# cudagu/aero-gnn

Measured on AMD Instinct MI355X. Metric: million edge-updates/sec, 1M-node/6M-edge mesh, 1->8 MI355X, higher is better.
Workload: dtype bf16; 1 GPU; BSMS-MGN 4-scale U-Net train step (fwd+MSE+bwd+allreduce+Adam), 1000000 nodes / 5996000 edges per GPU; model=BiStridedMeshGraphNet(H=128, n_hid=2, processor_size=15, stride=2, concat_trick), mode=train, global_batch=1, parallelism=dp1

## Files before the change

### aero-gnn_amd/aerognn/_lib.py

```python
from __future__ import annotations

import ctypes as C
import os

_HERE = os.path.dirname(os.path.abspath(__file__))
LIB_PATH = os.environ.get("AEROGNN_LIB") or os.path.join(_HERE, "libaerognn.so")

MAX_LIN = 8
MAX_SEG = 3
F32, BF16, F16, F64 = 0, 1, 2, 3
SEG_PLAIN, SEG_GATHER, SEG_SUM, SEG_MEAN = 0, 1, 2, 3
OPT_RESIDENT = 0

vp = C.c_void_p
i32 = C.c_int


class Seg(C.Structure):
    _fields_ = [("kind", i32), ("k", i32), ("ld", i32), ("_pad", i32),
                ("ptr", vp), ("index", vp), ("store", vp)]


ACT = {"relu": 0, "gelu": 1, "silu": 2, "tanh": 3}

# ... 34 lines not shown

class WgradBatch(C.Structure):
    _fields_ = [("n", i32), ("_pad", i32), ("d", WgradDesc * MAX_WGRAD)]


class WecArgs(C.Structure):
    _fields_ = [("n", i32), ("e", i32), ("dtype", i32), ("out_dim", i32), ("hid", i32), ("pos_dim", i32),
                ("pos_ld", i32), ("mean", i32),
                ("rowptr", vp), ("src", vp), ("dst", vp), ("perm", vp), ("rowptr_src", vp), ("perm_src", vp),
                ("pos", vp), ("pab", vp), ("tx", vp), ("w1c", vp), ("w2", vp),
                ("w_in", vp), ("w_out", vp), ("out", vp), ("dout", vp), ("gw", vp), ("s_csc", vp), ("dh", vp),
                ("dpa", vp), ("dpb", vp), ("dtx", vp), ("dw_in", vp), ("partial", vp)]


class EdgeBwdArgs(C.Structure):
    _fields_ = [("rows", i32), ("nblk", i32), ("wpk", vp * 4), ("bias", vp * 4), ("ln_g", vp), ("e", vp),
                ("proj", vp), ("src", vp), ("dst", vp), ("g", vp), ("g2", vp), ("de", vp), ("g0", vp),
                ("dw_partial", vp), ("db_partial", vp), ("ln_partial", vp), ("stamps", vp),
                ("a1", vp), ("stats", vp), ("scratch", vp), ("wtpk0", vp),
                ("xk", i32), ("xld", i32)]


class EdgeFwdArgs(C.Structure):
    _fields_ = [("rows", i32), ("nblk", i32), ("wpk", vp * 4), ("bias", vp * 4), ("ln_g", vp), ("ln_b", vp),
                ("e", vp), ("proj", vp), ("src", vp), ("dst", vp), ("out", vp), ("act", vp * 3), ("hpre", vp),
                ("stats", vp)]


class PackDesc(C.Structure):
    _fields_ = [("src", vp), ("dst", vp), ("src_dtype", i32), ("dst_dtype", i32),
                ("rows", i32), ("cols", i32), ("trans", i32), ("ld", i32),
                ("row_off", i32), ("col_off", i32), ("dst_rows", i32), ("dst_cols", i32)]


class F64Seg(C.Structure):
    _fields_ = [("a", vp), ("aidx", vp), ("lda", i32), ("k", i32), ("w", vp), ("ldw", i32), ("transw", i32)]


class F64GemmArgs(C.Structure):
    _fields_ = [("rows", i32), ("n", i32), ("nseg", i32), ("_pad", i32), ("seg", F64Seg * 3), ("bias", vp),
                ("add", vp * 2), ("add_idx", vp * 2), ("add_ld", i32 * 2), ("mask", vp), ("mask_ld", i32),
                ("relu", i32), ("out", vp), ("out_ld", i32), ("mask_act", i32), ("pre_out", vp),
                ("pre_ld", i32), ("_pad3", i32)]


class F64WgradArgs(C.Structure):
    _fields_ = [("rows", i32), ("m", i32), ("k", i32), ("_pad", i32), ("g", vp), ("ldg", i32), ("_pad1", i32),
                ("x", vp), ("ldx", i32), ("_pad2", i32), ("xidx", vp), ("dw", vp), ("ldw", i32), ("_pad3", i32),
                ("db", vp)]


_lib = None

LAUNCHES = ("agn_pack", "agn_mlp_forward", "agn_mlp_backward", "agn_reduce_partials", "agn_wgrad", "agn_colsum",
            "agn_segment_sum", "agn_segment_sum2", "agn_gather_rows", "agn_radix_sort_u64", "agn_row_ptr", "agn_row_ptr_i64",
            "agn_iota_keys", "agn_level_index",
            "agn_exclusive_scan_i32", "agn_pool_sort_keys", "agn_pool_assign", "agn_pool_edge_candidates",
            "agn_pool_edge_sort", "agn_pool_edge_emit", "agn_bfs_distance", "agn_center_seed", "agn_maxdeg_seed",
            "agn_bistride_select", "agn_index_map", "agn_subgraph_edges", "agn_scatter_rows", "agn_wec_forward",
            "agn_wec_backward", "agn_edge_features", "agn_node_features", "agn_normalize", "agn_col_stats", "agn_collate",
            "agn_segment_max", "agn_segment_max_backward", "agn_edge_bwd_fused", "agn_encoder_bwd_fused", "agn_wgrad_reduce",
            "agn_edge_forward32",
            "agn_proj_forward", "agn_proj_backward")


class AeroGNNError(RuntimeError):
    pass


class _Lib:

    def __init__(self, cdll):
        self._cdll = cdll
        for name in LAUNCHES:
            if hasattr(cdll, name):
                setattr(self, name, _timed_launch(getattr(cdll, name), name[4:]))

    def __getattr__(self, name):
        return getattr(self._cdll, name)


def _timed_launch(f, tag):
    from . import core

    def call(*args):
        prof = core.PROF
        if prof is None or core._TIMED_DEPTH:
            return f(*args)
        import torch
        s = torch.cuda.Event(enable_timing=True)
        s.record()
        rc = f(*args)
        e = torch.cuda.Event(enable_timing=True)
        e.record()
        prof.append((tag, None, s, e))
        return rc
    return call


def lib():
    global _lib
    if _lib is None:
        if not os.path.exists(LIB_PATH):
            raise AeroGNNError(
                f"{LIB_PATH} not found: build it with `make -C aero-gnn_amd/csrc` "
                "(or __graft_entry__.build()); the aerognn hot path has no CPU fallback")
        L = C.CDLL(LIB_PATH)
        sig = {
            "agn_version": (i32, []),
            "agn_error_string": (C.c_char_p, [i32]),
            "agn_set_option": (i32, [i32, i32]),
            "agn_packed_bytes": (C.c_size_t, [i32, i32, i32]),
            "agn_pack": (i32, [vp, i32, i32, vp]),
            "agn_mlp_forward": (i32, [C.POINTER(MlpFwdArgs), vp]),
            "agn_mlp_bwd_nwaves": (i32, [i32]),
            "agn_mlp_backward": (i32, [C.POINTER(MlpBwdArgs), vp]),
            "agn_reduce_partials": (i32, [vp, i32, i32, vp, vp]),
            "agn_wgrad_nsplit": (i32, [i32, i32]),
            "agn_wgrad_partial_floats": (C.c_size_t, [i32, i32, i32]),
            "agn_wgrad": (i32, [C.POINTER(WgradBatch), i32, i32, vp]),
            "agn_wgrad_plan": (i32, [C.POINTER(WgradBatch)]),
            "agn_colsum": (i32, [vp, i32, i32, vp, i32, vp, vp]),
            "agn_segment_sum": (i32, [i32, i32, i32, vp, vp, vp, i32, vp, i32, i32, vp]),
            "agn_segment_sum2": (i32, [i32, i32, i32, vp, i32, vp, vp, vp, i32, vp, vp, vp, i32, vp, i32, vp]),
            "agn_gather_rows": (i32, [i32, i32, i32, vp, vp, i32, vp, vp, i32, vp, i32, vp]),
            "agn_segment_max": (i32, [i32, i32, i32, vp, vp, vp, i32, vp, i32, vp, vp]),
            "agn_segment_max_backward": (i32, [i32, i32, i32, vp, vp, i32, vp, i32, vp]),
            "agn_radix_sort_temp_bytes": (C.c_size_t, [i32]),
            "agn_radix_sort_u64": (i32, [vp, vp, i32, i32, vp, vp, vp, vp]),
            "agn_row_ptr": (i32, [vp, i32, i32, vp, vp]),
            "agn_row_ptr_i64": (i32, [vp, i32, i32, vp, vp]),
            "agn_iota_keys": (i32, [i32, vp, vp, vp, vp, vp]),
            "agn_level_index": (i32, [i32, vp, C.c_int64, vp, vp, vp, vp, vp, vp, vp]),
            "agn_scan_temp_bytes": (C.c_size_t, [i32]),
            "agn_exclusive_scan_i32": (i32, [vp, vp, i32, vp, vp, vp]),
            "agn_pool_sort_keys": (i32, [i32, vp, vp, i32, vp, vp, vp]),
            "agn_pool_assign": (i32, [i32, i32, i32, vp, vp, vp, vp, i32, vp, vp, vp, vp, vp]),
            "agn_pool_edge_candidates": (i32, [i32, vp, vp, vp, vp, vp]),
            "agn_pool_edge_sort": (i32, [i32, vp, vp, vp, vp, vp, vp, vp, vp, vp, vp, vp]),
            "agn_pool_edge_emit": (i32, [i32, vp, vp, vp, vp, vp, vp, vp, vp, vp, vp, i32, vp]),
            "agn_bfs_work_ints": (C.c_size_t, [i32]),
            "agn_bfs_distance": (i32, [vp, vp, i32, i32, vp, vp, C.POINTER(i32), vp]),
            "agn_center_seed": (i32, [vp, i32, i32, i32, vp, vp]),
            "agn_maxdeg_seed": (i32, [vp, i32, vp, vp]),
            "agn_compact_work_ints": (C.c_size_t, [i32]),
            "agn_bistride_select": (i32, [vp, i32, vp, C.POINTER(i32), vp, vp]),
            "agn_index_map": (i32, [vp, i32, i32, vp, vp]),
            "agn_subgraph_edges": (i32, [vp, vp, i32, vp, vp, vp, C.POINTER(i32), vp, vp]),
            "agn_scatter_rows": (i32, [i32, i32, i32, vp, vp, i32, vp, i32, vp]),
            "agn_wec_blocks": (i32, [i32]),
            "agn_edge_bwd_blocks": (i32, [i32]),
            "agn_edge_bwd_scratch_bytes": (C.c_size_t, [i32]),
            "agn_edge_features": (i32, [i32, C.c_int64, i32, vp, vp, i32, vp, vp, vp, vp, vp]),
            "agn_normalize": (i32, [i32, i32, vp, i32, vp, vp, vp, i32, i32, vp]),
            "agn_col_stats_temp_bytes": (C.c_size_t, [i32, i32]),
            "agn_col_stats": (i32, [i32, i32, vp, i32, vp, vp, C.c_float, vp, vp]),
            "agn_collate": (i32, [i32, C.c_int64, C.c_int64, vp, vp, vp, vp, vp]),
            "agn_edge_bwd_fused": (i32, [C.POINTER(EdgeBwdArgs), vp]),
            "agn_encoder_bwd_fused": (i32, [C.POINTER(EdgeBwdArgs), vp]),
            "agn_edge_fwd32_blocks": (i32, [i32]),
            "agn_edge_forward32": (i32, [C.POINTER(EdgeFwdArgs), vp]),
            "agn_debug_node32_launches": (C.c_long, []),
            "agn_debug_enc32_launches": (C.c_long, []),
            "agn_debug_dec32_launches": (C.c_long, []),
            "agn_debug_node32_bwd_launches": (C.c_long, []),
            "agn_debug_dec32_bwd_launches": (C.c_long, []),
            "agn_fault_status": (i32, [C.POINTER(i32), i32]),
            "agn_fault_status_async": (i32, [vp, vp]),
            "agn_debug_set_fault": (i32, [i32]),
            "agn_wgrad_reduce": (i32, [C.POINTER(WgradBatch), i32, vp]),
            "agn_proj_forward": (i32, [i32, vp, i32, vp, vp, vp, i32, vp]),
            "agn_proj_backward": (i32, [i32, vp, vp, i32, vp, vp, i32, vp]),
            "agn_wec_forward": (i32, [C.POINTER(WecArgs), vp]),
            "agn_wec_backward": (i32, [C.POINTER(WecArgs), vp]),
# ... 39 lines not shown
```

### aero-gnn_amd/aerognn/core.py

```python
from __future__ import annotations

import ctypes as C

import torch

from . import _lib as L
from ._lib import check, ptr


def stream():
    return C.c_void_p(torch.cuda.current_stream().cuda_stream)


PROF = None
_TIMED_DEPTH = 0


class _Timed:
    __slots__ = ("tag", "cost", "s", "on")

    def __init__(self, tag, cost):
        self.tag, self.cost = tag, cost
        self.on = False

# ... 496 lines not shown
        self.tag = tag

    def add(self, G, X, dw, db=None, xidx=None):
        assert G.dtype == X.dtype and logical_rows(G) == (logical_rows(X) if xidx is None else xidx.numel())
        assert dw.dtype == torch.float32 and dw.stride(1) == 1
        assert xidx is None or (xidx.dtype == torch.int32 and not is_tiled(X))
        self.items.append((G, X, dw, db, xidx))

    def run(self):
        lib = L.lib()
        plain = [it for it in self.items if it[4] is None]
        gath = [it for it in self.items if it[4] is not None]
        chunks = [grp[i:i + L.MAX_WGRAD] for grp in (plain, gath) for i in range(0, len(grp), L.MAX_WGRAD)]
        for chunk in chunks:
            dev = chunk[0][0].device
            live = []
            for G, X, dw, db, xi in chunk:
                if logical_rows(G) == 0:
                    dw.zero_()
                    if db is not None:
                        db.zero_()
                else:
                    live.append((G, X, dw, db, xi))
            if not live:
                continue
            b = L.WgradBatch()
            b.n = len(live)
            for j, (G, X, dw, db, xi) in enumerate(live):
                b.d[j] = L.WgradDesc(ptr(G), ptr(X), G.stride(0), X.stride(0), G.shape[1], X.shape[1], logical_rows(G),
                                     dw.stride(0), None, None, ptr(dw), ptr(db), int(is_tiled(G)), int(is_tiled(X)), 0, 0,
                                     ptr(xi))
            check(lib.agn_wgrad_plan(C.byref(b)), "wgrad_plan")
            sizes = [int(lib.agn_wgrad_partial_floats(G.shape[1], X.shape[1], b.d[j].nsplit))
                     for j, (G, X, _, _, _) in enumerate(live)]
            bsz = [b.d[j].nsplit * ((G.shape[1] + 127) // 128) * 128 if db is not None else 0
                   for j, (G, _, _, db, _) in enumerate(live)]
            scratch = torch.empty(sum(sizes) + sum(bsz), dtype=torch.float32, device=dev)
            o = 0
            for j, (G, X, dw, db, _) in enumerate(live):
                b.d[j].dw_partial = ptr(scratch[o:o + sizes[j]])
                o += sizes[j]
                if db is not None:
                    b.d[j].db_partial = ptr(scratch[o:o + bsz[j]])
                    o += bsz[j]
            s_el = live[0][0].element_size()
            io = sum(logical_rows(G) * (G.shape[1] + X.shape[1]) * s_el + 4 * G.shape[1] * (X.shape[1] + 1)
                     for G, X, _, _, _ in live)
            fl = sum(2.0 * logical_rows(G) * G.shape[1] * X.shape[1] for G, X, _, _, _ in live)
            with timed(self.tag, (0.0, fl, io)):
                check(lib.agn_wgrad(C.byref(b), dt_code(live[0][0].dtype), 0, stream()), "wgrad")
        self.items = []


def alg8d_edge(E, N, H, s, bwd=False):
    return (2 if bwd else 1) * (E * (2 * s * H + 8) + N * 2 * s * H)


def alg8d_node(N, H, s, bwd=False, proj=False):
    return (2 if bwd else 1) * N * 3 * s * H * (2 if (bwd and proj) else 1)


def with_alg(alg, impl):
    return (alg, impl[1], impl[0])


def mask_bytes(H):
    return 8 * max(1, (H + 63) // 64)


def cost_edge_fwd(E, N, H, s, nlin, train, a1_saves=False):
    per = 2 * H * s + 8 + ((nlin - 1) * (H * s + mask_bytes(H)) + H * s + 8 if train else 0)
    per += (H * s + 8) if a1_saves else 0
    return E * per + N * 2 * H * s, 2 * E * H * H * nlin


def cost_node_fwd(E, N, H, s, nlin, train):
    per = 2 * H * s + 8 + ((nlin - 1) * (H * s + mask_bytes(H)) + 2 * H * s + 8 if train else 0)
    return N * per + E * H * s, 2 * N * H * (2 * H + (nlin - 1) * H)


def cost_proj(N, H, s):
    return N * 3 * H * s, 2 * N * H * 2 * H


def cost_edge_bwd(E, N, H, s, nlin):
    per = H * s + H * s + (nlin - 1) * mask_bytes(H) + H * s + 8 + nlin * H * s + H * s + 4
    return E * per + N * H * s, 2 * E * H * H * nlin


def cost_edge_fwd_cat(E, N, H, s, nlin, train):
    per = 4 * H * s + 8 + ((nlin - 1) * (H * s + mask_bytes(H)) + H * s + 8 if train else 0)
    return E * per, 2 * E * H * (3 * H + (nlin - 1) * H)


def cost_edge_bwd_cat(E, N, H, s, nlin):
    per = H * s + H * s + (nlin - 1) * mask_bytes(H) + H * s + 8 + nlin * H * s + 3 * H * s + 4
    return E * per + N * H * s, 2 * E * H * (3 * H + (nlin - 1) * H)


def cost_wec_fwd(E, N, out, s, hid=64):
    return E * (12 + hid * s + out * s + 24 + s) + N * (8 + hid * s + out * s), E * (2 * hid + 2 * out + 16)


def cost_wec_bwd(E, N, out, s, hid=64):
    dst = E * (12 + out * s + hid * s + 24 + 4 + 4 * hid) + N * (out * s + 2 * hid * s)
    src = E * (12 + out * s + 4 * hid) + N * (8 + out * s + hid * s)
# ... 16 lines not shown
```

### aero-gnn_amd/aerognn/functions.py

```python
from __future__ import annotations

import ctypes as C

import torch

from . import _lib as L
from ._lib import check, ptr
from . import core as _core
from .core import (Pack, WGrad, alg8d_edge, alg8d_node, with_alg, edge_bwd_fused, fused_edge_train_ok, bwd_nblocks,
                   edge32_ok, edge_saves_ok, edge_forward,
                   cost_edge_bwd_fused,
                   proj_kernel_ok, proj_forward, proj_backward, tiled_empty, relu_mask_empty, colsum_rows, cost_edge_bwd, cost_edge_bwd_cat, cost_edge_fwd,
                   cost_edge_fwd_cat, cost_node_bwd, cost_node_fwd, cost_proj, cost_wec_bwd, cost_wec_fwd, dt_code,
                   timed, gather_rows, mlp_backward, mlp_forward, require_device,
                   scatter_rows, segment_max, segment_max_backward, segment_sum, segment_sum2, stream)


def _c(t):
    return t if t.is_contiguous() else t.contiguous()


def _ln_grads(partial, nblk, M, dtype):
    out = torch.empty(2 * M, dtype=torch.float32, device=partial.device)
    colsum_rows(partial, nblk, 2 * M, out)
    return out[:M].to(dtype), out[M:].to(dtype)


class ChainSpec:

    def __init__(self, linears, ln, hidden, pack: Pack, prefix="", act="relu"):
        if act not in L.ACT:
            raise NotImplementedError(f"aerognn MLP kernels implement activation_fn in {sorted(L.ACT)}, got {act!r}")
        self.act = L.ACT[act]
        self.linears = linears
        self.ln = ln
        self.hidden = hidden
        self.nlin = len(linears)
        self.in_dim = linears[0][0].shape[1]
        self.out_dim = linears[-1][0].shape[0]
        self.tiled_saves = hidden == 128 and (ln is None or self.out_dim == hidden)
        self.p = prefix
        for l, (w, b) in enumerate(linears):
            M, K = w.shape
            pack.matrix(prefix + f"W{l}", M, K, [(w, 0, 0, False)])
            pack.matrix(prefix + f"T{l}", K, M, [(w, 0, 0, True)])
            if b is not None:
                pack.vector(prefix + f"b{l}", M, [(b, 0)])
        if ln is not None:
            pack.vector(prefix + "ln_g", ln[0].numel(), [(ln[0], 0)])
            pack.vector(prefix + "ln_b", ln[1].numel(), [(ln[1], 0)])
        self.pack = pack

    def wpk(self):
        return [self.pack[self.p + f"W{l}"] for l in range(self.nlin)]

    def wtpk(self):
        return [self.pack[self.p + f"T{l}"] for l in range(self.nlin)]

    def biases(self):
        return [self.pack[self.p + f"b{l}"] if self.linears[l][1] is not None else None for l in range(self.nlin)]

    def lnp(self):
        return (self.pack[self.p + "ln_g"], self.pack[self.p + "ln_b"]) if self.ln is not None else None

    def params(self):
# ... 367 lines not shown
    def backward(ctx, gx, ge):
        x, e = ctx.saved_tensors
        spec, lv = ctx.spec, ctx.level
        ea, ehp, est, na, nhp, nst, agg = ctx.saves
        es, ns = spec.edge, spec.node
        dt, dev = x.dtype, x.device
        N, E, H = x.shape[0], e.shape[0], spec.H
        gx = _c(gx) if gx is not None else torch.zeros_like(x)
        ge = _c(ge) if ge is not None else None
        gpre_n = _alloc_gpre(ns, N, dt, dev)
        dx = torch.empty_like(x)
        dagg = torch.empty(N, H, dtype=dt, device=dev)
        nb_n = bwd_nblocks(N)
        part_n = torch.empty(nb_n, 2 * H, dtype=torch.float32, device=dev) if ns.ln else None
        nb_n = mlp_backward(rows=N, dtype=dt, hidden=H, nlin=ns.nlin, act_fn=ns.act, out_dim=H, in_dim=2 * H, wtpk=ns.wtpk(),
                     acts=na, g=gx, gpre=gpre_n, ln_g=ns.lnp()[0] if ns.ln else None, hpre=nhp, stats=nst,
                     din=[(H, dx, True), (H, dagg, False)], ln_partial=part_n,
                     tag="node_bwd", cost=with_alg(alg8d_node(N, H, x.element_size(), bwd=True, proj=spec.trick),
                                                   cost_node_bwd(N, H, x.element_size(), ns.nlin)))
        if spec.aggregation == "mean":
            dagg = gather_rows(N, H, None, dagg, torch.empty_like(dagg), cnt_ptr=lv.rowptr)
        fused = ctx.fused
        de = torch.empty_like(e)
        sz = x.element_size()
        if fused:
            g0 = torch.empty(E, H, dtype=dt, device=dev)
            a1s, sts = ctx.esaves
            dW13, db13, part_e, nb_e = edge_bwd_fused(
                rows=E, wpk=es.wpk(), wtpk0=es.wtpk()[0], bias=es.biases(), ln_g=es.lnp()[0], e=e, proj=ctx.proj, src=lv.src, dst=lv.dst,
                g=ge, g2=dagg, de=de, g0=g0, tag="edge_bwd", a1=a1s, stats=sts,
                cost=with_alg(alg8d_edge(E, N, H, sz, bwd=True), cost_edge_bwd_fused(E, N, H, sz, saved=a1s is not None)))
        else:
            nb_e = bwd_nblocks(E)
            part_e = torch.empty(nb_e, 2 * H, dtype=torch.float32, device=dev) if es.ln else None
            gpre_e = _alloc_gpre(es, E, dt, dev, rowmajor=(0,) if spec.trick else ())
            if spec.trick:
                din = [(H, de, True)]
            else:
                dxs = torch.empty(E, H, dtype=dt, device=dev)
                dxd = torch.empty(E, H, dtype=dt, device=dev)
                din = [(H, dxs, False), (H, dxd, False), (H, de, True)] if spec.gmp_order else \
                    [(H, de, True), (H, dxs, False), (H, dxd, False)]
            nb_e = mlp_backward(rows=E, dtype=dt, hidden=H, nlin=es.nlin, act_fn=es.act, out_dim=H, in_dim=es.in_dim,
                                wtpk=es.wtpk(), acts=ea, g=ge, g2=dagg, gidx=lv.dst, gpre=gpre_e,
                                ln_g=es.lnp()[0] if es.ln else None, hpre=ehp, stats=est, din=din, ln_partial=part_e,
                                tag="edge_bwd",
                                cost=with_alg(alg8d_edge(E, N, H, sz, bwd=True),
                                              (cost_edge_bwd if spec.trick else cost_edge_bwd_cat)(E, N, H, sz,
                                                                                                   es.nlin)))
            g0 = gpre_e[0]
        grads_edge = []
        if spec.trick:
            dPs = segment_sum(N, H, lv.rowptr_src, lv.perm_src, g0, torch.empty(N, H, dtype=dt, device=dev))
            dPd = segment_sum(N, H, lv.rowptr, None, g0, torch.empty(N, H, dtype=dt, device=dev))
            if proj_kernel_ok(dx, H):
                s_el = dx.element_size()
                proj_backward(N, dPs, dPd, spec.pack["projT"], dx, tag="proj_bwd",
                              cost=with_alg(alg8d_node(N, H, s_el, bwd=True), (4 * N * H * s_el, 4.0 * N * H * H)))
            else:
                mlp_forward(rows=N, dtype=dt, hidden=H, nlin=1, out_dim=H,
                            segs=[(L.SEG_PLAIN, H, H, dPs, None, None), (L.SEG_PLAIN, H, H, dPd, None, None)],
                            wpk=[spec.pack["projT"]], bias=[None], resid=dx, out=dx)
            eb = spec.eb
            wg = WGrad("wgrad_node")
            if fused:
                dwe = torch.empty(H, H, dtype=torch.float32, device=dev)
                we = WGrad("wgrad_edge")
                we.add(g0, e, dwe)
                we.run()
                eg = [dwe]
                for l in range(3):
                    eg += [dW13[l], db13[l]]
                eg = eg[:1] + [t if t.dtype == p.dtype else t.to(p.dtype) for t, p in zip(eg[1:], es.params()[1:7])]
                eg += list(_ln_grads(part_e, nb_e, H, es.ln[0].dtype))
            else:
                eg = _chain_param_grads(es, gpre_e, e, ea, part_e, nb_e, tag="wgrad_edge")
            dws = torch.empty(H, x.shape[1], dtype=torch.float32, device=dev)
            dwd = torch.empty(H, x.shape[1], dtype=torch.float32, device=dev)
            dbd = torch.empty(H, dtype=torch.float32, device=dev)
            wg.add(dPs, x, dws)
            wg.add(dPd, x, dwd, dbd)
            grads_node = _chain_param_grads(ns, gpre_n, [x, agg], na, part_n, nb_n, wg)
            wg.run()
            if fused and eg[0].dtype != es.linears[0][0].dtype:
                eg[0] = eg[0].to(es.linears[0][0].dtype)
            grads_edge = [eg[0], dws.to(eb.src_lin.dtype), dwd.to(eb.dst_lin.dtype), dbd.to(eb.bias.dtype)] + eg[1:]
            return (dx, de, None, None, None, *grads_edge, *grads_node)
        else:
            segment_sum2(N, H, dx, (lv.rowptr_src, lv.perm_src, dxs), (lv.rowptr, None, dxd), dx)
            xs, xd = (x, lv.src), (x, lv.dst)
            grads_edge = _chain_param_grads(es, gpre_e, [xs, xd, e] if spec.gmp_order else [e, xs, xd],
                                            ea, part_e, nb_e, tag="wgrad_edge")
        grads_node = _chain_param_grads(ns, gpre_n, [x, agg], na, part_n, nb_n, tag="wgrad_node")
        return (dx, de, None, None, None, *grads_edge, *grads_node)


class GradBox:
    __slots__ = ("g", "armed")

    def __init__(self):
        self.g = None
        self.armed = False

    def put(self, g):
        self.g = g if self.g is None else self.g + g

    def take(self):
        if self.armed and self.g is None:
            raise RuntimeError("aerognn: skip gradient missing (autograd order violated)")
        g, self.g = self.g, None
        return g


class SkipFn(torch.autograd.Function):

    @staticmethod
    def forward(ctx, t, box):
        box.armed = True
        ctx.box = box
        return t.view_as(t)

    @staticmethod
# ... 467 lines not shown
```

### aero-gnn_amd/csrc/dw.hip

```cpp
#include "common.hpp"
#include "host.hpp"
#include "aerognn.h"

#include <type_traits>

using namespace agn;

namespace {

#ifndef AGN_DW_ROWS
#define AGN_DW_ROWS 64
#endif
constexpr int DW_ROWS = AGN_DW_ROWS;
constexpr int DW_BLK = 128;
constexpr int DW_THREADS = 256;

typedef short s16x4 __attribute__((ext_vector_type(4)));
typedef __attribute__((address_space(3))) s16x4 lds_s16x4;

template <typename T> struct DwTile;
template <> struct DwTile<bf16> { static constexpr int LD = 136; };
template <> struct DwTile<f16> { static constexpr int LD = 136; };
template <> struct DwTile<float> { static constexpr int LD = 132; };

// ... 62 lines not shown
            v[j] = __builtin_bit_cast(uint4, u32x4{lo[0], lo[1], hi[0], hi[1]});
          } else {
            T e8[PER16];
#pragma unroll
            for (int e = 0; e < PER16; ++e) e8[e] = e < nv ? p[e] : from_f<T>(0.f);
            v[j] = *reinterpret_cast<const uint4*>(e8);
          }
        }
      }
    }
  }
  AGN_DEV void store(T* lds, int tiled) const {
    constexpr int LD = DwTile<T>::LD;
    if (tiled) {
#pragma unroll
      for (int j = 0; j < NCH; ++j) {
        int row, i, hh;
        tiled_pos(threadIdx.x + j * DW_THREADS, row, i, hh);
        if constexpr (sizeof(T) == 2) {
          const u32x4 x = __builtin_bit_cast(u32x4, v[j]);
          typedef uint32_t u32x2 __attribute__((ext_vector_type(2)));
          *reinterpret_cast<u32x2*>(lds + row * LD + 16 * i + 4 * hh) = u32x2{x[0], x[1]};
          *reinterpret_cast<u32x2*>(lds + row * LD + 16 * i + 8 + 4 * hh) = u32x2{x[2], x[3]};
        } else {
          *reinterpret_cast<uint4*>(lds + row * LD + 8 * i + 4 * hh) = v[j];
        }
      }
      return;
    }
#pragma unroll
    for (int j = 0; j < NCH; ++j) {
      const int i = threadIdx.x + j * DW_THREADS;
      const int r = i / CHUNKS, ch = i - r * CHUNKS;
      *reinterpret_cast<uint4*>(lds + r * LD + ch * PER16) = v[j];
    }
  }
};

AGN_DEV bf16x8 tr_frag(const bf16* lds, int kb, int col_base, int lane) {
  constexpr int LD = DwTile<bf16>::LD;
  const int q = (lane & 15) >> 2, p = lane & 3;
  const bf16* a0 = lds + (kb + q) * LD + col_base + 4 * p;
  const bf16* a1 = a0 + 4 * LD;
  s16x4 lo = __builtin_amdgcn_ds_read_tr16_b64_v4i16((lds_s16x4*)(a0));
  s16x4 hi = __builtin_amdgcn_ds_read_tr16_b64_v4i16((lds_s16x4*)(a1));
  bf16x8 r;
  const bf16x4 l4 = *reinterpret_cast<const bf16x4*>(&lo);
  const bf16x4 h4 = *reinterpret_cast<const bf16x4*>(&hi);
  r[0] = l4[0]; r[1] = l4[1]; r[2] = l4[2]; r[3] = l4[3];
  r[4] = h4[0]; r[5] = h4[1]; r[6] = h4[2]; r[7] = h4[3];
  return r;
}

template <typename T, bool XG>
__global__ __launch_bounds__(DW_THREADS) void wgrad_kernel(const agn_wgrad_batch b, int nsplit) {
  constexpr int LD = DwTile<T>::LD;
  __shared__ __attribute__((aligned(16))) T sg[DW_ROWS * LD];
  __shared__ __attribute__((aligned(16))) T sx[DW_ROWS * LD];
  const agn_wgrad_desc& d = b.d[blockIdx.z];
  const int nKb = (d.k + DW_BLK - 1) / DW_BLK;
  const int nMb = (d.m + DW_BLK - 1) / DW_BLK;
  if ((int)blockIdx.y >= nMb * nKb) return;
  const int mb = blockIdx.y / nKb, kb = blockIdx.y % nKb;
  const int m0 = mb * DW_BLK, k0 = kb * DW_BLK;
  const int split = blockIdx.x;
  const int per = ((d.rows + nsplit - 1) / nsplit + DW_ROWS - 1) / DW_ROWS * DW_ROWS;
  const int rbeg = split * per, rend = min(d.rows, rbeg + per);
  const int lane = threadIdx.x & 63, w = threadIdx.x >> 6;
  const int wm = (w >> 1) * 64, wk = (w & 1) * 64;
  const T* G = reinterpret_cast<const T*>(d.g);
  const T* X = reinterpret_cast<const T*>(d.x);
  f32x16 acc[2][2];
#pragma unroll
  for (int i = 0; i < 2; ++i)
#pragma unroll
    for (int j = 0; j < 2; ++j) acc[i][j] = f32x16{};
  float bsum = 0.f;
  __shared__ float bhalf[DW_BLK];
  StageRegs<T> rg, rx;
  if (rbeg < rend) {
    rg.load(G, d.ldg, rend, d.m, rbeg, m0, d.g_tiled);
    rx.load(X, d.ldx, rend, d.k, rbeg, k0, d.x_tiled, XG ? d.xidx : nullptr);
  }
  for (int r0 = rbeg; r0 < rend; r0 += DW_ROWS) {
    __syncthreads();
    rg.store(sg, d.g_tiled);
    rx.store(sx, d.x_tiled);
    __syncthreads();
    if (r0 + DW_ROWS < rend) {
      rg.load(G, d.ldg, rend, d.m, r0 + DW_ROWS, m0, d.g_tiled);
      rx.load(X, d.ldx, rend, d.k, r0 + DW_ROWS, k0, d.x_tiled, XG ? d.xidx : nullptr);
    }
    if (d.db_partial && kb == 0) {
      const int col = threadIdx.x & (DW_BLK - 1), q = threadIdx.x >> 7;
#pragma unroll
      for (int gq = 0; gq < DW_ROWS / 32; ++gq)
#pragma unroll 8
        for (int r = 0; r < 16; ++r) bsum += to_f(sg[(32 * gq + 16 * q + r) * LD + col]);
    }
    if constexpr (sizeof(T) == 2) {
#pragma unroll
      for (int ks = 0; ks < DW_ROWS; ks += 16) {
        const int kbase = ks + 8 * (lane >> 5);
        bf16x8 a[2], bb[2];
#pragma unroll
        for (int i = 0; i < 2; ++i) a[i] = tr_frag(reinterpret_cast<const bf16*>(sg), kbase, wm + 32 * i + 16 * ((lane >> 4) & 1), lane);
#pragma unroll
        for (int j = 0; j < 2; ++j) bb[j] = tr_frag(reinterpret_cast<const bf16*>(sx), kbase, wk + 32 * j + 16 * ((lane >> 4) & 1), lane);
#pragma unroll
        for (int i = 0; i < 2; ++i)
#pragma unroll
          for (int j = 0; j < 2; ++j) {
            if constexpr (std::is_same<T, f16>::value)
              acc[i][j] = __builtin_amdgcn_mfma_f32_32x32x16_f16(__builtin_bit_cast(f16x8, a[i]),
                                                                 __builtin_bit_cast(f16x8, bb[j]), acc[i][j], 0, 0, 0);
            else
              acc[i][j] = __builtin_amdgcn_mfma_f32_32x32x16_bf16(a[i], bb[j], acc[i][j], 0, 0, 0);
          }
      }
    } else {
      const float* fg = reinterpret_cast<const float*>(sg);
      const float* fx = reinterpret_cast<const float*>(sx);
#pragma unroll 4
      for (int ks = 0; ks < DW_ROWS; ks += 2) {
        const int r = ks + (lane >> 5), cidx = lane & 31;
        float a[2], bb[2];
#pragma unroll
        for (int i = 0; i < 2; ++i) a[i] = fg[r * LD + wm + 32 * i + cidx];
#pragma unroll
        for (int j = 0; j < 2; ++j) bb[j] = fx[r * LD + wk + 32 * j + cidx];
#pragma unroll
        for (int i = 0; i < 2; ++i)
#pragma unroll
          for (int j = 0; j < 2; ++j) acc[i][j] = __builtin_amdgcn_mfma_f32_32x32x2f32(a[i], bb[j], acc[i][j], 0, 0, 0);
      }
    }
  }
  const int kpad = nKb * DW_BLK;
  float* P = d.dw_partial + (size_t)split * (nMb * DW_BLK) * kpad;
#pragma unroll
  for (int i = 0; i < 2; ++i)
#pragma unroll
    for (int j = 0; j < 2; ++j)
#pragma unroll
      for (int r = 0; r < 16; ++r) {
        const int m = m0 + wm + 32 * i + (r & 3) + 8 * (r >> 2) + 4 * (lane >> 5);
        const int k = k0 + wk + 32 * j + (lane & 31);
        P[(size_t)m * kpad + k] = acc[i][j][r];
      }
  if (d.db_partial && kb == 0) {
    __syncthreads();
    if (threadIdx.x >= DW_BLK) bhalf[threadIdx.x - DW_BLK] = bsum;
    __syncthreads();
    if (threadIdx.x < DW_BLK) d.db_partial[(size_t)split * (nMb * DW_BLK) + m0 + threadIdx.x] = bsum + bhalf[threadIdx.x];
  }
}

constexpr int RED_G = 8;
constexpr int RED_Q = 16;
__global__ __launch_bounds__(RED_Q * RED_G) void wgrad_reduce_kernel(const agn_wgrad_batch b) {
  __shared__ f32x4 part[RED_G][RED_Q];
  __shared__ float bpart[RED_G][RED_Q];
  const agn_wgrad_desc& d = b.d[blockIdx.y];
  const int nsplit = d.nsplit;
  const int nKb = (d.k + DW_BLK - 1) / DW_BLK, nMb = (d.m + DW_BLK - 1) / DW_BLK;
  const int kpad = nKb * DW_BLK, mpad = nMb * DW_BLK;
  const size_t slab = (size_t)mpad * kpad;
  const int kq = kpad / 4;
  const int t = threadIdx.x % RED_Q, g = threadIdx.x / RED_Q;
  const int qidx = blockIdx.x * RED_Q + t;
  const bool in_slab = qidx < mpad * kq;
  f32x4 s = {0.f, 0.f, 0.f, 0.f};
  if (in_slab) {
    const float* p = d.dw_partial + (size_t)qidx * 4;
    int sp = g;
    for (; sp + 3 * RED_G < nsplit; sp += 4 * RED_G) {
      f32x4 v[4];
#pragma unroll
      for (int j = 0; j < 4; ++j) v[j] = *reinterpret_cast<const f32x4*>(p + (size_t)(sp + j * RED_G) * slab);
#pragma unroll
      for (int j = 0; j < 4; ++j) {
        s[0] += v[j][0]; s[1] += v[j][1]; s[2] += v[j][2]; s[3] += v[j][3];
      }
    }
    for (; sp < nsplit; sp += RED_G) {
      const f32x4 v = *reinterpret_cast<const f32x4*>(p + (size_t)sp * slab);
      s[0] += v[0]; s[1] += v[1]; s[2] += v[2]; s[3] += v[3];
    }
  }
  part[g][t] = s;
// ... 88 lines not shown

int agn_wgrad_nsplit(int rows, int ndesc_blocks) {
  int ns = wgrad_resident() / (ndesc_blocks > 0 ? ndesc_blocks : 1);
  const int maxs = (rows + 2 * DW_ROWS - 1) / (2 * DW_ROWS);
  if (ns > maxs) ns = maxs;
  return ns < 1 ? 1 : ns;
}

size_t agn_wgrad_partial_floats(int m, int k, int nsplit) {
  const int mp = (m + DW_BLK - 1) / DW_BLK * DW_BLK, kp = (k + DW_BLK - 1) / DW_BLK * DW_BLK;
  return (size_t)nsplit * mp * kp;
}

int agn_wgrad_plan(agn_wgrad_batch* b) {
  if (!b || b->n < 1 || b->n > AGN_MAX_WGRAD) return AGN_E_ARG;
  int nblk = 0, rows = 0;
  for (int i = 0; i < b->n; ++i) {
    nblk += out_blocks(b->d[i]);
    rows = b->d[i].rows > rows ? b->d[i].rows : rows;
  }
  const int ns = agn_wgrad_nsplit(rows, nblk);
  for (int i = 0; i < b->n; ++i) b->d[i].nsplit = ns;
  return 0;
}

int agn_wgrad(const agn_wgrad_batch* b, int dtype, int nsplit, void* stream) {
  if (!b || b->n < 1 || b->n > AGN_MAX_WGRAD) return AGN_E_ARG;
  agn_wgrad_batch bb = *b;
  int total = 0, maxq = 1;
  for (int i = 0; i < bb.n; ++i) {
    agn_wgrad_desc& d = bb.d[i];
    if (d.m < 1 || d.k < 1 || d.rows < 0) return AGN_E_ARG;
    if ((d.g_tiled && d.m != DW_BLK) || (d.x_tiled && d.k != DW_BLK)) return AGN_E_SHAPE;
    if (d.xidx && d.x_tiled) return AGN_E_ARG;
    if (nsplit > 0) d.nsplit = nsplit;
    if (d.nsplit < 1) return AGN_E_ARG;
    total += out_blocks(d) * d.nsplit;
    const int kpad = ((d.k + DW_BLK - 1) / DW_BLK) * DW_BLK, mpad = ((d.m + DW_BLK - 1) / DW_BLK) * DW_BLK;
    maxq = mpad * kpad / 4 > maxq ? mpad * kpad / 4 : maxq;
  }
  hipStream_t st = (hipStream_t)stream;
  const int ns = bb.d[0].nsplit;
  int maxblk = 1;
  for (int i = 0; i < bb.n; ++i) {
    if (bb.d[i].nsplit != ns) return AGN_E_ARG;
    maxblk = out_blocks(bb.d[i]) > maxblk ? out_blocks(bb.d[i]) : maxblk;
  }
  (void)total;
  dim3 grid(ns, maxblk, bb.n);
  bool xg = false;
  for (int i = 0; i < bb.n; ++i) xg = xg || bb.d[i].xidx != nullptr;
#define AGN_WG(T)                                                                             \
  do {                                                                                        \
    if (xg) hipLaunchKernelGGL((wgrad_kernel<T, true>), grid, dim3(DW_THREADS), 0, st, bb, ns); \
    else hipLaunchKernelGGL((wgrad_kernel<T, false>), grid, dim3(DW_THREADS), 0, st, bb, ns);   \
  } while (0)
  if (dtype == AGN_BF16) AGN_WG(bf16);
  else if (dtype == AGN_F16) AGN_WG(f16);
  else if (dtype == AGN_F32) AGN_WG(float);
  else return AGN_E_DTYPE;
#undef AGN_WG
  hipLaunchKernelGGL(wgrad_reduce_kernel, dim3((maxq + RED_Q - 1) / RED_Q, bb.n), dim3(RED_Q * RED_G), 0, st, bb);
  return launch_status();
}

int agn_wgrad_reduce(const agn_wgrad_batch* b, int nsplit, void* stream) {
  if (!b || b->n < 1 || b->n > AGN_MAX_WGRAD || nsplit < 1) return AGN_E_ARG;
  agn_wgrad_batch bb = *b;
  int maxq = 1;
  for (int i = 0; i < bb.n; ++i) {
    bb.d[i].nsplit = nsplit;
    const int kpad = ((bb.d[i].k + DW_BLK - 1) / DW_BLK) * DW_BLK;
    const int mpad = ((bb.d[i].m + DW_BLK - 1) / DW_BLK) * DW_BLK;
    maxq = mpad * kpad / 4 > maxq ? mpad * kpad / 4 : maxq;
  }
  hipLaunchKernelGGL(wgrad_reduce_kernel, dim3((maxq + RED_Q - 1) / RED_Q, bb.n), dim3(RED_Q * RED_G), 0, (hipStream_t)stream, bb);
  return launch_status();
}

int agn_colsum(const float* p, int nw, int n, float* scratch, int scratch_rows, float* out, void* stream) {
  if (nw < 0 || n < 1 || scratch_rows < 1) return AGN_E_ARG;
  hipStream_t st = (hipStream_t)stream;
  if (nw == 0) {
    hipError_t e = hipMemsetAsync(out, 0, sizeof(float) * n, st);
    return e == hipSuccess ? 0 : (int)e;
  }
  const int chunk = (nw + scratch_rows - 1) / scratch_rows;
  const int nc = (nw + chunk - 1) / chunk;
  hipLaunchKernelGGL(colsum_stage1, dim3((n + 255) / 256, nc), dim3(256), 0, st, p, nw, n, chunk, scratch);
  hipLaunchKernelGGL(colsum_stage2, dim3((n + 63) / 64), dim3(64 * RED_G), 0, st, scratch, nc, n, out);
  return launch_status();
}

}
```

### include/aerognn.h

```cpp
#ifndef AEROGNN_H
#define AEROGNN_H
#include <stddef.h>
#include <stdint.h>
#ifdef __cplusplus
extern "C" {
#endif

#define AGN_MAX_LIN 8
#define AGN_MAX_SEG 3

enum { AGN_F32 = 0, AGN_BF16 = 1, AGN_F16 = 2, AGN_F64 = 3 };
enum { AGN_SEG_PLAIN = 0, AGN_SEG_GATHER = 1, AGN_SEG_SUM = 2, AGN_SEG_MEAN = 3 };
enum { AGN_E_ARG = -1, AGN_E_DTYPE = -2, AGN_E_HIDDEN = -3, AGN_E_SHAPE = -4 };
enum { AGN_ACT_RELU = 0, AGN_ACT_GELU = 1, AGN_ACT_SILU = 2, AGN_ACT_TANH = 3 };

typedef struct {
  int kind;
  int k;
  int ld;
  int _pad;
  const void* ptr;
  const int32_t* index;
  void* store;
} agn_seg;
// ... 49 lines not shown
  void* din[AGN_MAX_SEG];
  int din_resid[AGN_MAX_SEG];
  float* ln_partial;
  int tiled;
  int gpre_tiled;
  const void* mask[AGN_MAX_LIN];
  int act_fn;
  int _pad3;
  const void* pre[AGN_MAX_LIN];
} agn_mlp_bwd_args;



typedef struct {
  const void* src;
  void* dst;
  int src_dtype;
  int dst_dtype;
  int rows;
  int cols;
  int trans;
  int ld;
  int row_off;
  int col_off;
  int dst_rows;
  int dst_cols;
} agn_pack_desc;

#define AGN_MAX_WGRAD 8
typedef struct {
  const void* g;
  const void* x;
  int ldg, ldx;
  int m, k, rows;
  int ldw;
  float* dw_partial;
  float* db_partial;
  float* dw;
  float* db;
  int g_tiled, x_tiled;
  int nsplit;
  int _pad;
  const int32_t* xidx;
} agn_wgrad_desc;
typedef struct {
  int n;
  int _pad;
  agn_wgrad_desc d[AGN_MAX_WGRAD];
} agn_wgrad_batch;
int agn_wgrad_nsplit(int rows, int ndesc_blocks);
size_t agn_wgrad_partial_floats(int m, int k, int nsplit);
int agn_wgrad_plan(agn_wgrad_batch* b);
int agn_wgrad(const agn_wgrad_batch* b, int dtype, int nsplit, void* stream);
int agn_colsum(const float* p, int nw, int n, float* scratch, int scratch_rows, float* out, void* stream);

int agn_version(void);
const char* agn_error_string(int code);
enum {
  AGN_OPT_RESIDENT = 0
};
int agn_set_option(int key, int value);
size_t agn_packed_bytes(int m, int k, int dtype);
int agn_pack(const agn_pack_desc* descs_device, int n, int max_threads, void* stream);

int agn_mlp_forward(const agn_mlp_fwd_args* a, void* stream);
int agn_mlp_bwd_nwaves(int rows);
int agn_mlp_backward(const agn_mlp_bwd_args* a, void* stream);
int agn_reduce_partials(const float* partial, int nw, int n, float* out, void* stream);

int agn_segment_sum(int rows, int k, int dtype, const int32_t* ptr, const int32_t* perm,
                    const void* src, int src_ld, void* out, int out_ld, int mean, void* stream);
int agn_segment_sum2(int rows, int k, int dtype, const void* base, int base_ld, const int32_t* ptr_a,
                     const int32_t* perm_a, const void* src_a, int lda, const int32_t* ptr_b,
                     const int32_t* perm_b, const void* src_b, int ldb, void* out, int out_ld, void* stream);
int agn_segment_max(int rows, int k, int dtype, const int32_t* ptr, const int32_t* perm, const void* src,
                    int src_ld, void* out, int out_ld, int32_t* argmax, void* stream);
int agn_segment_max_backward(int rows, int k, int dtype, const int32_t* argmax, const void* gout, int gout_ld,
                             void* dx, int dx_ld, void* stream);
int agn_gather_rows(int rows, int k, int dtype, const int32_t* idx, const void* src, int src_ld,
                    const int32_t* cnt_ptr, const void* add, int add_ld, void* out, int out_ld,
                    void* stream);

size_t agn_radix_sort_temp_bytes(int n);
int agn_radix_sort_u64(uint64_t* keys, int32_t* vals, int n, int bits, uint64_t* keys_tmp,
                       int32_t* vals_tmp, void* scratch, void* stream);
int agn_row_ptr(const int32_t* sorted_keys, int n, int nrows, int32_t* ptr, void* stream);

size_t agn_scan_temp_bytes(int n);
int agn_exclusive_scan_i32(const int32_t* in, int32_t* out, int n, int32_t* total, int32_t* scratch,
                           void* stream);
int agn_iota_keys(int n, const int32_t* keys32, const int64_t* keys64, int64_t* keys, int32_t* vals, void* stream);
int agn_level_index(int e, const int64_t* edge_index, int64_t ld, const int32_t* perm, int32_t* src, int32_t* dst,
                    int64_t* perm64, int64_t* inv64, int32_t* inv32, void* stream);
int agn_row_ptr_i64(const int64_t* sorted_keys, int n, int nrows, int32_t* ptr, void* stream);

int agn_pool_sort_keys(int n, const int64_t* batch, const float* pos, int pos_ld, uint64_t* keys,
                       int32_t* vals, void* stream);
int agn_pool_assign(int n, int nc, int ngraph, const int64_t* batch, const int32_t* sorted_nodes,
                    const int32_t* gstart, const int32_t* coff, int stride, int32_t* f2c,
                    int32_t* c2f, int32_t* c2f_ptr, int64_t* cbatch, void* stream);
int agn_pool_edge_candidates(int nc, const int32_t* c2f, const int32_t* c2f_ptr, const int32_t* rowptr,
                             int32_t* cand_cnt, void* stream);
int agn_pool_edge_sort(int nc, const int32_t* c2f, const int32_t* c2f_ptr, const int32_t* rowptr,
                       const int32_t* src, const int64_t* refkey, const int32_t* f2c,
                       const int32_t* cand_ptr, int32_t* cand_tmp, int32_t* cand_sorted,
                       int32_t* uniq, void* stream);
// ... 170 lines not shown
```

Before: 788.7 M edge-updates/s.

## Fuse destination segment-sum into edge weight-gradient kernel sharing staged g0 tiles

When the concat trick is active, the backward pass now computes the destination-node segment sum of g0 inside the edge weight-gradient kernel instead of launching a separate segment_sum. The fused kernel walks CSR row pointers while g0 tiles are already staged in shared memory, so g0 (E x 128) is read from HBM once rather than twice. It adds a segment-walker state machine, drains leftover segments from global memory, and raises the launch-bounds occupancy hint for the fused variant. The trade-off is extra register pressure and per-wave serial segment handling, which may slow the GEMM part.

```diff
diff --git a/aero-gnn_amd/aerognn/_lib.py b/aero-gnn_amd/aerognn/_lib.py
--- a/aero-gnn_amd/aerognn/_lib.py
+++ b/aero-gnn_amd/aerognn/_lib.py
@@ -110,7 +110,7 @@
 
 _lib = None
 
-LAUNCHES = ("agn_pack", "agn_mlp_forward", "agn_mlp_backward", "agn_reduce_partials", "agn_wgrad", "agn_colsum",
+LAUNCHES = ("agn_pack", "agn_mlp_forward", "agn_mlp_backward", "agn_reduce_partials", "agn_wgrad", "agn_wgrad_segsum", "agn_colsum",
             "agn_segment_sum", "agn_segment_sum2", "agn_gather_rows", "agn_radix_sort_u64", "agn_row_ptr", "agn_row_ptr_i64",
             "agn_iota_keys", "agn_level_index",
             "agn_exclusive_scan_i32", "agn_pool_sort_keys", "agn_pool_assign", "agn_pool_edge_candidates",
@@ -178,6 +178,8 @@
             "agn_wgrad_partial_floats": (C.c_size_t, [i32, i32, i32]),
             "agn_wgrad": (i32, [C.POINTER(WgradBatch), i32, i32, vp]),
             "agn_wgrad_plan": (i32, [C.POINTER(WgradBatch)]),
+            "agn_wgrad_segsum": (i32, [C.POINTER(WgradBatch), i32, i32, vp, vp, i32, vp, i32, vp]),
+            "agn_debug_wgrad_occupancy": (i32, [i32]),
             "agn_colsum": (i32, [vp, i32, i32, vp, i32, vp, vp]),
             "agn_segment_sum": (i32, [i32, i32, i32, vp, vp, vp, i32, vp, i32, i32, vp]),
             "agn_segment_sum2": (i32, [i32, i32, i32, vp, i32, vp, vp, vp, i32, vp, vp, vp, i32, vp, i32, vp]),
diff --git a/aero-gnn_amd/aerognn/core.py b/aero-gnn_amd/aerognn/core.py
--- a/aero-gnn_amd/aerognn/core.py
+++ b/aero-gnn_amd/aerognn/core.py
@@ -572,6 +572,37 @@
         self.items = []
 
 
+def wgrad_dpd_ok(g, x):
+    import os
+    return (os.environ.get("AEROGNN_WG_DPD", "1") != "0" and g.dtype in (torch.bfloat16, torch.float16)
+            and g.dtype == x.dtype and g.dim() == 2 and x.dim() == 2 and g.shape[1] == 128 and x.shape[1] == 128
+            and g.stride(1) == 1 and x.stride(1) == 1 and not is_tiled(g) and not is_tiled(x))
+
+
+def wgrad_segsum(G, X, dw, rowptr, dst, out, tag="wgrad_edge"):
+    lib = L.lib()
+    rows, N = G.shape[0], out.shape[0]
+    assert X.shape[0] == rows and rowptr.dtype == torch.int32 and rowptr.numel() == N + 1
+    assert dst.dtype == torch.int32 and dst.numel() == rows and dst.is_contiguous() and rowptr.is_contiguous()
+    assert dw.dtype == torch.float32 and dw.stride(1) == 1 and out.dtype == G.dtype and out.stride(1) == 1
+    b = L.WgradBatch()
+    b.n = 1
+    b.d[0] = L.WgradDesc(ptr(G), ptr(X), G.stride(0), X.stride(0), 128, 128, rows, dw.stride(0), None, None, ptr(dw),
+                         None, 0, 0, 0, 0, None)
+    scratch = None
+    if rows > 0:
+        check(lib.agn_wgrad_plan(C.byref(b)), "wgrad_plan")
+        scratch = torch.empty(int(lib.agn_wgrad_partial_floats(128, 128, b.d[0].nsplit)), dtype=torch.float32,
+                              device=G.device)
+        b.d[0].dw_partial = ptr(scratch)
+    s_el = G.element_size()
+    io = rows * 256 * s_el + 4 * 128 * 129 + N * 128 * s_el + 4 * (N + 1)
+    with timed(tag, (0.0, 2.0 * rows * 128 * 128, io)):
+        check(lib.agn_wgrad_segsum(C.byref(b), dt_code(G.dtype), 0, ptr(rowptr), ptr(dst), N, ptr(out), out.stride(0), stream()),
+              "wgrad_segsum")
+    return out
+
+
 def alg8d_edge(E, N, H, s, bwd=False):
     return (2 if bwd else 1) * (E * (2 * s * H + 8) + N * 2 * s * H)
 
diff --git a/aero-gnn_amd/aerognn/functions.py b/aero-gnn_amd/aerognn/functions.py
--- a/aero-gnn_amd/aerognn/functions.py
+++ b/aero-gnn_amd/aerognn/functions.py
@@ -10,7 +10,7 @@
 from .core import (Pack, WGrad, alg8d_edge, alg8d_node, with_alg, edge_bwd_fused, fused_edge_train_ok, bwd_nblocks,
                    edge32_ok, edge_saves_ok, edge_forward,
                    cost_edge_bwd_fused,
-                   proj_kernel_ok, proj_forward, proj_backward, tiled_empty, relu_mask_empty, colsum_rows, cost_edge_bwd, cost_edge_bwd_cat, cost_edge_fwd,
+                   proj_kernel_ok, proj_forward, proj_backward, wgrad_dpd_ok, wgrad_segsum, tiled_empty, relu_mask_empty, colsum_rows, cost_edge_bwd, cost_edge_bwd_cat, cost_edge_fwd,
                    cost_edge_fwd_cat, cost_node_bwd, cost_node_fwd, cost_proj, cost_wec_bwd, cost_wec_fwd, dt_code,
                    timed, gather_rows, mlp_backward, mlp_forward, require_device,
                    scatter_rows, segment_max, segment_max_backward, segment_sum, segment_sum2, stream)
@@ -484,7 +484,13 @@
         grads_edge = []
         if spec.trick:
             dPs = segment_sum(N, H, lv.rowptr_src, lv.perm_src, g0, torch.empty(N, H, dtype=dt, device=dev))
-            dPd = segment_sum(N, H, lv.rowptr, None, g0, torch.empty(N, H, dtype=dt, device=dev))
+            dPd = torch.empty(N, H, dtype=dt, device=dev)
+            dwe = None
+            if fused and wgrad_dpd_ok(g0, e):
+                dwe = torch.empty(H, H, dtype=torch.float32, device=dev)
+                wgrad_segsum(g0, e, dwe, lv.rowptr, lv.dst, dPd)
+            else:
+                segment_sum(N, H, lv.rowptr, None, g0, dPd)
             if proj_kernel_ok(dx, H):
                 s_el = dx.element_size()
                 proj_backward(N, dPs, dPd, spec.pack["projT"], dx, tag="proj_bwd",
@@ -496,10 +502,11 @@
             eb = spec.eb
             wg = WGrad("wgrad_node")
             if fused:
-                dwe = torch.empty(H, H, dtype=torch.float32, device=dev)
-                we = WGrad("wgrad_edge")
-                we.add(g0, e, dwe)
-                we.run()
+                if dwe is None:
+                    dwe = torch.empty(H, H, dtype=torch.float32, device=dev)
+                    we = WGrad("wgrad_edge")
+                    we.add(g0, e, dwe)
+                    we.run()
                 eg = [dwe]
                 for l in range(3):
                     eg += [dW13[l], db13[l]]
diff --git a/aero-gnn_amd/csrc/dw.hip b/aero-gnn_amd/csrc/dw.hip
--- a/aero-gnn_amd/csrc/dw.hip
+++ b/aero-gnn_amd/csrc/dw.hip
@@ -138,8 +138,95 @@
   return r;
 }
 
-template <typename T, bool XG>
-__global__ __launch_bounds__(DW_THREADS) void wgrad_kernel(const agn_wgrad_batch b, int nsplit) {
+struct WgSeg {
+  const int32_t* ptr;
+  const int32_t* dst;
+  int n;
+  void* out;
+  int out_ld;
+};
+
+template <typename T>
+struct SegWalk {
+  typedef const __attribute__((address_space(4))) int32_t* cptr_t;
+  cptr_t ptr, dst;
+  int rows;
+  int n, nhi;
+  int cur, end;
+  bool open;
+  float s0, s1;
+
+  AGN_DEV int at(int i) const { return min(max(ptr[i], 0), rows); }
+  AGN_DEV int first_from(int cnt, int r) const {
+    int i = min(max(dst[r], 0), cnt - 1);
+    if (at(i) < r) return i + 1;
+    while (i > 0 && at(i - 1) >= r) --i;
+    return i;
+  }
+  AGN_DEV void init(const WgSeg& sa, int rows_, int rbeg, int per, int wave) {
+    ptr = (cptr_t)(uintptr_t)sa.ptr;
+    dst = (cptr_t)(uintptr_t)sa.dst;
+    rows = rows_;
+    n = nhi = 0;
+    cur = end = 0;
+    open = false;
+    s0 = s1 = 0.f;
+    if (rbeg >= rows || sa.n < 1) return;
+    const int nlo = first_from(sa.n, rbeg);
+    nhi = per >= rows - rbeg ? sa.n : first_from(sa.n, rbeg + per);
+    n = nlo + ((wave - nlo) & 3);
+  }
+  AGN_DEV bool next() {
+    if (n >= nhi) return false;
+    cur = at(n);
+    end = max(cur, at(n + 1));
+    s0 = s1 = 0.f;
+    open = true;
+    return true;
+  }
+  AGN_DEV void add_rows(const T* p, size_t ld, int base, int from, int stop, int lane) {
+    for (int r = from; r < stop; r += 4) {
+      uint32_t v[4];
+#pragma unroll
+      for (int q = 0; q < 4; ++q)
+        v[q] = *reinterpret_cast<const uint32_t*>(reinterpret_cast<const char*>(p + (size_t)(min(r + q, stop - 1) - base) * ld) +
+                                                  (uint32_t)(4 * lane));
+#pragma unroll
+      for (int q = 0; q < 4; ++q)
+        if (r + q < stop) {
+          s0 += lo16<T>(v[q]);
+          s1 += hi16<T>(v[q]);
+        }
+    }
+  }
+  AGN_DEV void finish(const WgSeg& sa, int lane) {
+    *reinterpret_cast<uint32_t*>(reinterpret_cast<char*>(reinterpret_cast<T*>(sa.out) + (size_t)n * sa.out_ld) +
+                                 (uint32_t)(4 * lane)) = pack2t<T>(s0, s1);
+    open = false;
+    n += 4;
+  }
+  AGN_DEV void stage(const WgSeg& sa, const T* sg, int ld, int r0, int se, int lane) {
+    for (;;) {
+      if (!open && !next()) break;
+      if (cur < end && cur >= se) break;
+      const int stop = min(end, se);
+      add_rows(sg, ld, r0, max(cur, r0), stop, lane);
+      cur = max(cur, stop);
+      if (cur < end) break;
+      finish(sa, lane);
+    }
+  }
+  AGN_DEV void drain(const WgSeg& sa, const T* G, int ldg, int lane) {
+    for (;;) {
+      if (!open && !next()) break;
+      add_rows(G, ldg, 0, cur, end, lane);
+      finish(sa, lane);
+    }
+  }
+};
+
+template <typename T, bool XG, bool SEG = false>
+__global__ __launch_bounds__(DW_THREADS, SEG ? 3 : 1) void wgrad_kernel(const agn_wgrad_batch b, int nsplit, const WgSeg sa) {
   constexpr int LD = DwTile<T>::LD;
   __shared__ __attribute__((aligned(16))) T sg[DW_ROWS * LD];
   __shared__ __attribute__((aligned(16))) T sx[DW_ROWS * LD];
@@ -164,10 +251,12 @@
   float bsum = 0.f;
   __shared__ float bhalf[DW_BLK];
   StageRegs<T> rg, rx;
+  SegWalk<typename std::conditional<SEG, T, bf16>::type> walk;
   if (rbeg < rend) {
     rg.load(G, d.ldg, rend, d.m, rbeg, m0, d.g_tiled);
     rx.load(X, d.ldx, rend, d.k, rbeg, k0, d.x_tiled, XG ? d.xidx : nullptr);
   }
+  if constexpr (SEG) walk.init(sa, d.rows, rbeg, per, __builtin_amdgcn_readfirstlane(w));
   for (int r0 = rbeg; r0 < rend; r0 += DW_ROWS) {
     __syncthreads();
     rg.store(sg, d.g_tiled);
@@ -177,6 +266,7 @@
       rg.load(G, d.ldg, rend, d.m, r0 + DW_ROWS, m0, d.g_tiled);
       rx.load(X, d.ldx, rend, d.k, r0 + DW_ROWS, k0, d.x_tiled, XG ? d.xidx : nullptr);
     }
+    if constexpr (SEG) walk.stage(sa, sg, LD, r0, min(r0 + DW_ROWS, rend), lane);
     if (d.db_partial && kb == 0) {
       const int col = threadIdx.x & (DW_BLK - 1), q = threadIdx.x >> 7;
 #pragma unroll
@@ -222,6 +312,7 @@
       }
     }
   }
+  if constexpr (SEG) walk.drain(sa, G, d.ldg, lane);
   const int kpad = nKb * DW_BLK;
   float* P = d.dw_partial + (size_t)split * (nMb * DW_BLK) * kpad;
 #pragma unroll
@@ -416,8 +507,8 @@
   for (int i = 0; i < bb.n; ++i) xg = xg || bb.d[i].xidx != nullptr;
 #define AGN_WG(T)                                                                             \
   do {                                                                                        \
-    if (xg) hipLaunchKernelGGL((wgrad_kernel<T, true>), grid, dim3(DW_THREADS), 0, st, bb, ns); \
-    else hipLaunchKernelGGL((wgrad_kernel<T, false>), grid, dim3(DW_THREADS), 0, st, bb, ns);   \
+    if (xg) hipLaunchKernelGGL((wgrad_kernel<T, true>), grid, dim3(DW_THREADS), 0, st, bb, ns, WgSeg{}); \
+    else hipLaunchKernelGGL((wgrad_kernel<T, false>), grid, dim3(DW_THREADS), 0, st, bb, ns, WgSeg{});   \
   } while (0)
   if (dtype == AGN_BF16) AGN_WG(bf16);
   else if (dtype == AGN_F16) AGN_WG(f16);
@@ -426,6 +517,40 @@
 #undef AGN_WG
   hipLaunchKernelGGL(wgrad_reduce_kernel, dim3((maxq + RED_Q - 1) / RED_Q, bb.n), dim3(RED_Q * RED_G), 0, st, bb);
   return launch_status();
+}
+
+int agn_wgrad_segsum(const agn_wgrad_batch* b, int dtype, int nsplit, const int32_t* rowptr, const int32_t* dst, int n,
+                     void* out, int out_ld, void* stream) {
+  if (!b || b->n != 1 || n < 0 || (n > 0 && (!rowptr || !out))) return AGN_E_ARG;
+  if (dtype != AGN_BF16 && dtype != AGN_F16) return AGN_E_DTYPE;
+  agn_wgrad_batch bb = *b;
+  agn_wgrad_desc& d = bb.d[0];
+  if (d.rows < 0 || !d.dw) return AGN_E_ARG;
+  if (d.m != DW_BLK || d.k != DW_BLK || d.g_tiled || d.x_tiled || d.xidx || d.db || d.db_partial) return AGN_E_SHAPE;
+  if (out_ld < DW_BLK || (out_ld & 1) || (reinterpret_cast<uintptr_t>(out) & 3)) return AGN_E_SHAPE;
+  hipStream_t st = (hipStream_t)stream;
+  if (d.rows == 0) {
+    hipError_t e = hipMemset2DAsync(d.dw, sizeof(float) * d.ldw, 0, sizeof(float) * d.k, d.m, st);
+    if (e == hipSuccess && n > 0) e = hipMemset2DAsync(out, (size_t)2 * out_ld, 0, (size_t)2 * DW_BLK, n, st);
+    return e == hipSuccess ? 0 : (int)e;
+  }
+  if (!dst || n < 1) return AGN_E_ARG;
+  if (!d.g || !d.x || !d.dw_partial || (d.ldg & 1) || (reinterpret_cast<uintptr_t>(d.g) & 3)) return AGN_E_SHAPE;
+  if (nsplit > 0) d.nsplit = nsplit;
+  if (d.nsplit < 1) return AGN_E_ARG;
+  const int ns = d.nsplit;
+  const WgSeg sa{rowptr, dst, n, out, out_ld};
+  if (dtype == AGN_BF16) hipLaunchKernelGGL((wgrad_kernel<bf16, false, true>), dim3(ns, 1, 1), dim3(DW_THREADS), 0, st, bb, ns, sa);
+  else hipLaunchKernelGGL((wgrad_kernel<f16, false, true>), dim3(ns, 1, 1), dim3(DW_THREADS), 0, st, bb, ns, sa);
+  hipLaunchKernelGGL(wgrad_reduce_kernel, dim3((DW_BLK * DW_BLK / 4 + RED_Q - 1) / RED_Q, 1), dim3(RED_Q * RED_G), 0, st, bb);
+  return launch_status();
+}
+
+int agn_debug_wgrad_occupancy(int segsum) {
+  int per = 0;
+  const hipError_t e = segsum ? hipOccupancyMaxActiveBlocksPerMultiprocessor(&per, wgrad_kernel<bf16, false, true>, DW_THREADS, 0)
+                              : hipOccupancyMaxActiveBlocksPerMultiprocessor(&per, wgrad_kernel<bf16, false>, DW_THREADS, 0);
+  return e == hipSuccess ? per : 0;
 }
 
 int agn_wgrad_reduce(const agn_wgrad_batch* b, int nsplit, void* stream) {
diff --git a/include/aerognn.h b/include/aerognn.h
--- a/include/aerognn.h
+++ b/include/aerognn.h
@@ -125,6 +125,9 @@
 size_t agn_wgrad_partial_floats(int m, int k, int nsplit);
 int agn_wgrad_plan(agn_wgrad_batch* b);
 int agn_wgrad(const agn_wgrad_batch* b, int dtype, int nsplit, void* stream);
+int agn_wgrad_segsum(const agn_wgrad_batch* b, int dtype, int nsplit, const int32_t* rowptr, const int32_t* dst, int n,
+                     void* out, int out_ld, void* stream);
+int agn_debug_wgrad_occupancy(int segsum);
 int agn_colsum(const float* p, int nw, int n, float* scratch, int scratch_rows, float* out, void* stream);
 
 int agn_version(void);
```

Result: faster. 802.4 M edge-updates/s, median of 6 (+1.7%).
